# ai4ce/V2X-Sim

Measured on AMD Instinct MI355X. Metric: BEV frames/sec, V2VNet 5-agent detection (256x256 BEV), higher is better.
Workload: dtype bf16

## Files before the change

### v2x-sim_amd/csrc/api.hip

```cpp
#include "common.h"
#include <cxxabi.h>
#include <dlfcn.h>
#include <stdlib.h>
#include <string.h>

static thread_local char g_err[512] = "";

void v2x_set_error(const char *fmt, ...) {
    va_list ap;
    va_start(ap, fmt);
    vsnprintf(g_err, sizeof(g_err), fmt, ap);
    va_end(ap);
}

extern "C" __attribute__((weak)) int v2x_probe_build_marker;
extern "C" int v2x_abi_version(void) { return &v2x_probe_build_marker != nullptr ? -V2X_AMD_ABI_VERSION : V2X_AMD_ABI_VERSION; }

struct v2x_launch_plan { char *buf; size_t cap, len; };
__thread v2x_launch_plan *v2x_plan_sink = nullptr;

int v2x_plan_record(const void *kernel, const char *what) {
    v2x_launch_plan &p = *v2x_plan_sink;
    Dl_info info;
    char *dem = nullptr;
// ... 11 lines not shown
            else if (b[i] == '(' && --depth == 0) { n = i; break; }
        }
    }
    const size_t sep = p.len ? 3 : 0;
    const bool fits = p.len + sep + n + 1 <= p.cap;
    if (fits) {
        memcpy(p.buf + p.len, " + ", sep);
        memcpy(p.buf + p.len + sep, b, n);
        p.len += sep + n;
        p.buf[p.len] = 0;
    }
    free(dem);
    V2X_REQUIRE(fits, "v2x_conv2d_plan: the kernel names do not fit %zu bytes", p.cap);
    return V2X_OK;
}

extern "C" int v2x_conv2d_plan(const v2x_conv_desc *d, char *buf, size_t cap) {
    V2X_REQUIRE(buf && cap > 0, "v2x_conv2d_plan: no buffer");
    buf[0] = 0;
    v2x_launch_plan plan = {buf, cap, 0};
    v2x_plan_sink = &plan;
    const int rc = v2x_conv2d(d, nullptr);
    v2x_plan_sink = nullptr;
    return rc;
}

#include <atomic>
#include <mutex>
#include <strings.h>
namespace {
struct TuneEntry { const char *name; int def; };
const TuneEntry kTune[V2X_TUNE_COUNT] = {
    {"STREAM_WAVES", 8}, {"STREAM_G", 1}, {"STREAM_WT", 1}, {"STORE_X4", 1}, {"STREAM_PERSIST", 1}, {"STREAM_WIDE", 1},
    {"WIDE3", 1}, {"HALO_PP", 1}, {"VOXELIZE_LDS", 1}, {"WARP_LDS", 2}, {"S2_G", 1}, {"GRU_XCD_WALK", 1}, {"HALO_XCD", 1}, {"WGRAD_TR", 1}, {"BN_PARTIAL_T", 1}, {"WGRAD_REDUCE4", 1}, {"CONV1X1", 1},
};
std::atomic<int> g_tune[V2X_TUNE_COUNT];
std::once_flag g_tune_once;
void tune_init() {
    for (int i = 0; i < V2X_TUNE_COUNT; ++i) {
        char env[64];
        snprintf(env, sizeof(env), "V2X_%s", kTune[i].name);
        const char *e = getenv(env);
        g_tune[i].store((e && *e) ? atoi(e) : kTune[i].def, std::memory_order_relaxed);
    }
}
int tune_find(const char *name) {
    if (!name) return -1;
    if (strncasecmp(name, "V2X_", 4) == 0) name += 4;
    for (int i = 0; i < V2X_TUNE_COUNT; ++i)
        if (strcasecmp(name, kTune[i].name) == 0) return i;
    return -1;
}
}

int v2x_tune(int id) {
    std::call_once(g_tune_once, tune_init);
    return g_tune[id].load(std::memory_order_relaxed);
}
extern "C" int v2x_tuning_set(const char *name, int value) {
    const int i = tune_find(name);
    V2X_REQUIRE(i >= 0, "v2x_tuning_set: unknown switch '%s'", name ? name : "(null)");
    std::call_once(g_tune_once, tune_init);
    g_tune[i].store(value, std::memory_order_relaxed);
    return V2X_OK;
}
extern "C" int v2x_tuning_get(const char *name, int *value) {
    const int i = tune_find(name);
// ... 6 lines not shown
```

### v2x-sim_amd/csrc/common.h

```cpp
#pragma once
#include <hip/hip_runtime.h>
#include <stdint.h>
#include <stdio.h>
#include <stdarg.h>

#include "../../include/v2x_amd.h"

typedef __attribute__((ext_vector_type(8))) __bf16 bf16x8_t;
typedef __attribute__((ext_vector_type(4))) float f32x4_t;
typedef __attribute__((ext_vector_type(16))) float f32x16_t;

void v2x_set_error(const char *fmt, ...);

enum v2x_tune_id {
    V2X_TUNE_STREAM_WAVES,
    V2X_TUNE_STREAM_G,
    V2X_TUNE_STREAM_WT,
    V2X_TUNE_STORE_X4,
    V2X_TUNE_STREAM_PERSIST,
    V2X_TUNE_STREAM_WIDE,
    V2X_TUNE_WIDE3,
    V2X_TUNE_HALO_PP,
    V2X_TUNE_VOXELIZE_LDS,
    V2X_TUNE_WARP_LDS,
    V2X_TUNE_S2_G,
    V2X_TUNE_GRU_XCD_WALK,
    V2X_TUNE_HALO_XCD,
    V2X_TUNE_WGRAD_TR,
    V2X_TUNE_BN_PARTIAL_T,
    V2X_TUNE_WGRAD_REDUCE4,
    V2X_TUNE_CONV1X1,
    V2X_TUNE_COUNT
};
int v2x_tune(int id);

#define V2X_REQUIRE(cond, ...)            \
    do {                                  \
        if (!(cond)) {                    \
            v2x_set_error(__VA_ARGS__);   \
            return V2X_EINVAL;            \
        }                                 \
    } while (0)

#define V2X_CHECK_LAUNCH(name)                                                   \
    do {                                                                         \
        hipError_t e_ = hipGetLastError();                                       \
        if (e_ != hipSuccess) {                                                  \
            v2x_set_error("%s: launch failed: %s", name, hipGetErrorString(e_)); \
            return V2X_EIO;                                                      \
        }                                                                        \
    } while (0)

#define V2X_MAX_DEVICES 32
struct v2x_once_per_device { bool done[V2X_MAX_DEVICES]; };
static inline bool v2x_first_use_on_device(v2x_once_per_device &o) {
    int dev = 0;
    if (hipGetDevice(&dev) != hipSuccess || dev < 0 || dev >= V2X_MAX_DEVICES) return true;
    if (o.done[dev]) return false;
    o.done[dev] = true;
    return true;
}

struct v2x_launch_plan;
extern __thread v2x_launch_plan *v2x_plan_sink;
// ... 72 lines not shown
```

### v2x-sim_amd/csrc/conv_stream_pc.hip

```cpp
#include "conv_stream.h"

namespace pcs {
constexpr int TH = 16, TW = 32, BCO = 128, TCO = 8, HCO = 4;
constexpr int PW0 = TW / 2 + 2, PH0 = TH / 2 + 2;
constexpr int PHF = TH + 2, PWH = (TW + 2) / 2;
constexpr int SLICE = BCO * 64;
constexpr int USTEP = 4 * SLICE, SSTEP = 3 * SLICE;
constexpr int UP_PIECES = (PH0 * PW0 * 4 + 63) / 64;
constexpr int SP_PIECES = (2 * PHF * PWH * 4 + 63) / 64;
#ifndef V2X_PCS_USLOTS_BUILD
#define V2X_PCS_USLOTS_BUILD 3
#endif
constexpr int NU = V2X_PCS_USLOTS_BUILD;
constexpr int OFF_P0 = 3 * SSTEP, OFF_P1 = OFF_P0 + SP_PIECES * 1024;
constexpr int OFF_UPA = NU * USTEP, OFF_UPB = OFF_UPA + UP_PIECES * 1024;
constexpr int OFF_SS = (OFF_UPB + UP_PIECES * 1024 > OFF_P1 + SP_PIECES * 1024) ? OFF_UPB + UP_PIECES * 1024 : OFF_P1 + SP_PIECES * 1024;
constexpr int SMEM = OFF_SS + 2 * BCO * 4;
static_assert(SMEM <= 160 * 1024 && (NU == 3 || NU == 4), "LDS map");
#define PCS_SWZ(pc) (((pc) >> 1) & 3)

}

__global__ __launch_bounds__(512) __attribute__((amdgpu_waves_per_eu(2, 2))) void conv3x3_stream8p_kernel(const StreamArgs a) {
    using namespace pcs;
    extern __shared__ __attribute__((aligned(16))) char smem[];
    const int tid = threadIdx.x;
    const int lane = tid & 63;
    const int wave = __builtin_amdgcn_readfirstlane(tid >> 6);
    const int grp = wave >> 2, wv = wave & 3;
    const int py = wv >> 1, px = wv & 1;
    const int fj = lane & 15, fq = lane >> 4;

    const int nwg = gridDim.x;
    int bid = blockIdx.x;
    {
        const int q = nwg >> 3, r = nwg & 7, xcd = bid & 7, i = bid >> 3;
        bid = (xcd < r ? xcd * (q + 1) : r * (q + 1) + (xcd - r) * q) + i;
    }
    const int n_tiles = a.n_px_tiles * a.n_co_tiles;
    const int co_tile = bid % a.n_co_tiles;
    const int txy = a.tiles_x * a.tiles_y;
    const int n_up = a.C0 >> 5, n_sk = a.C1 >> 5;
    const int S_up = 4 * n_up, S_sk = 3 * n_sk;
    const size_t tile_bytes = (size_t)S_up * USTEP + (size_t)S_sk * SSTEP;
    const char *w_up = reinterpret_cast<const char *>(a.w) + (size_t)co_tile * tile_bytes;
    const char *w_sk = w_up + (size_t)S_up * USTEP;
    const void *zero_page = reinterpret_cast<const char *>(a.w) + (size_t)a.n_co_tiles * tile_bytes;
    const int Hs = a.H >> 1, Ws = a.W >> 1;

    auto tile_coords = [&](int t, int &n, int &y0, int &x0) {
        const int px_tile = t / a.n_co_tiles;
        n = px_tile / txy;
        const int trem = px_tile - n * txy;
        const int ty = trem / a.tiles_x;
        y0 = ty * TH;
        x0 = (trem - ty * a.tiles_x) * TW;
    };
    auto fresh_lane = [&]() -> int {
        int l;
        asm volatile("v_mbcnt_lo_u32_b32 %0, -1, 0\n\tv_mbcnt_hi_u32_b32 %0, -1, %0" : "=v"(l));
        return l;
    };
    auto issue_up_patch_piece = [&](int n, int y0, int x0, int kc, int piece, int buf_off) {
        const int L = piece * 64 + fresh_lane();
// ... 7 lines not shown
    auto issue_sk_patch_piece = [&](int n, int y0, int x0, int kc, int piece, int buf_off) {
        const int L = piece * 64 + fresh_lane();
        const int pix = L >> 2, phys = L & 3;
        const int q = pix / (PHF * PWH), rem = pix - q * (PHF * PWH);
        const int pr = rem / PWH, cc = rem - pr * PWH;
        const int y = y0 - 1 + pr, x = x0 - 1 + 2 * cc + q;
        const bool ok = pix < 2 * PHF * PWH && (unsigned)y < (unsigned)a.H && (unsigned)x < (unsigned)a.W;
        const unsigned off = (unsigned)((n * a.H + y) * a.W + x) * (unsigned)a.C1 + (unsigned)(kc * 32 + ((phys ^ PCS_SWZ(cc)) << 3));
        glds16s(ok ? (const void *)(a.in1 + off) : zero_page, smem + buf_off + piece * 1024);
    };
    auto issue_up_weights = [&](int st, int first, int count) {
        const int lane_w = fresh_lane();
        const char *src = w_up + (size_t)st * USTEP + lane_w * 16;
        char *dst = smem + (st % NU) * USTEP;
#pragma unroll
        for (int u = 0; u < 12; ++u)
            if (u < count) glds16s(src + (first + u) * 1024, dst + (first + u) * 1024);
    };
    auto issue_sk_weights = [&](int st, int first, int count) {
        const int lane_w = fresh_lane();
        const char *src = w_sk + (size_t)st * SSTEP + lane_w * 16;
        char *dst = smem + (st % 3) * SSTEP;
#pragma unroll
        for (int u = 0; u < 6; ++u)
            if (u < count) glds16s(src + (first + u) * 1024, dst + (first + u) * 1024);
    };
    auto up_buf = [&](int kc) { return ((n_up - 1 - kc) & 1) ? OFF_UPB : OFF_UPA; };
    auto sk_buf = [&](int kc) { return (kc & 1) ? OFF_P0 : OFF_P1; };
    auto up_prologue = [&](int n, int y0, int x0) {
        if (grp == 0) {
#pragma unroll
            for (int u = 0; u < 3; ++u) issue_up_patch_piece(n, y0, x0, 0, wv + 4 * u, up_buf(0));
        }
        if constexpr (NU == 3) {
            issue_up_weights(wave >> 2, (wave & 3) * 8, 8);
        } else {
            issue_up_weights((wave * 12) / 32, (wave * 12) % 32, ((wave * 12) % 32 + 12 <= 32) ? 12 : 32 - (wave * 12) % 32);
            if ((wave * 12) % 32 + 12 > 32) issue_up_weights((wave * 12) / 32 + 1, 0, (wave * 12) % 32 + 12 - 32);
        }
    };

    float *s_ss = reinterpret_cast<float *>(smem + OFF_SS);
    for (int i = tid; i < BCO; i += 512) {
        const int co = co_tile * BCO + i;
        s_ss[i] = co < a.Cout ? a.scale[co] : 0.f;
        s_ss[BCO + i] = co < a.Cout ? a.shift[co] : 0.f;
    }
    const uint32_t floor_bits = a.relu ? 0u : 0x80008000u;

    int tile = bid;
    int n, y0, x0;
    tile_coords(tile, n, y0, x0);
    up_prologue(n, y0, x0);
    asm volatile("s_waitcnt vmcnt(0) lgkmcnt(0)" ::: "memory");

    for (;;) {
        const int next = tile + nwg;
        const bool has_next = next < n_tiles;
        f32x4_t acc[TCO][4];
#pragma unroll
        for (int i = 0; i < TCO; ++i)
#pragma unroll
            for (int f = 0; f < 4; ++f) acc[i][f] = (f32x4_t)(0.f);

        __builtin_amdgcn_s_barrier();
        if (grp == 1) __builtin_amdgcn_s_barrier();
        for (int kc = 0; kc < n_up; ++kc) {
            const char *pb = smem + up_buf(kc);
#pragma unroll
            for (int t = 0; t < 4; ++t) {
                const int st = kc * 4 + t;
                const int ta = t >> 1, tb = t & 1;
                const int ln = fresh_lane();
                const int fjl = ln & 15, fql = ln >> 4;
                [[maybe_unused]] int nw = 0;
                if (grp == 1) {
                    if (st + NU - 1 < S_up) {
                        issue_up_weights(st + NU - 1, wv * 8, 8);
                        nw = 8;
                    }
                } else if (t < 3 && kc + 1 < n_up) {
                    issue_up_patch_piece(n, y0, x0, kc + 1, wv + 4 * t, up_buf(kc + 1));
                }
                __builtin_amdgcn_sched_barrier(0);
                bf16x8_t B[4], A[TCO];
                {
                    const int pc = fjl + tb + px;
                    const char *p = pb + ((4 * grp + py + ta) * PW0 * 4 + pc * 4 + (fql ^ PCS_SWZ(pc))) * 16;
#pragma unroll
                    for (int y = 0; y < 4; ++y) B[y] = *reinterpret_cast<const bf16x8_t *>(p + y * (PW0 * 64));
                    const char *ws = smem + (st % NU) * USTEP + wv * SLICE + (fql * BCO + fjl) * 16;
#pragma unroll
                    for (int i = 0; i < TCO; ++i) A[i] = *reinterpret_cast<const bf16x8_t *>(ws + i * 256);
                }
                __builtin_amdgcn_s_waitcnt(0xc07f);
                if (grp == 1) {
                    int keep = 0;
                    for (int d = 2; d <= NU - 1; ++d) keep += (st + d < S_up) ? 8 : 0;
                    const int stores = (st < NU - 2) ? (a.x4 ? 16 : 32) : 0;
                    switch (keep + stores) {
                        case 8: asm volatile("s_waitcnt vmcnt(8)" ::: "memory"); break;
                        case 16: asm volatile("s_waitcnt vmcnt(16)" ::: "memory"); break;
                        case 24: asm volatile("s_waitcnt vmcnt(24)" ::: "memory"); break;
                        case 32: asm volatile("s_waitcnt vmcnt(32)" ::: "memory"); break;
                        case 40: asm volatile("s_waitcnt vmcnt(40)" ::: "memory"); break;
                        case 48: asm volatile("s_waitcnt vmcnt(48)" ::: "memory"); break;
                        default: asm volatile("s_waitcnt vmcnt(0)" ::: "memory"); break;
                    }
                } else if (t == 3) {
                    asm volatile("s_waitcnt vmcnt(0)" ::: "memory");
                }
                __builtin_amdgcn_sched_barrier(0);
                __builtin_amdgcn_s_barrier();
                __builtin_amdgcn_sched_barrier(0);
#pragma unroll
                for (int i = 0; i < TCO; ++i)
#pragma unroll
                    for (int y = 0; y < 4; ++y) acc[i][y] = __builtin_amdgcn_mfma_f32_16x16x32_bf16(A[i], B[y], acc[i][y], 0, 0, 0);
                __builtin_amdgcn_sched_barrier(0);
                __builtin_amdgcn_s_barrier();
                __builtin_amdgcn_sched_barrier(0);
            }
        }
        if (grp == 0) __builtin_amdgcn_s_barrier();

        if (grp == 0) {
#pragma unroll
            for (int u = 0; u < 10; ++u)
                if (wv + 4 * u < SP_PIECES) issue_sk_patch_piece(n, y0, x0, 0, wv + 4 * u, sk_buf(0));
        }
        issue_sk_weights(wave >> 2, (wave & 3) * 6, 6);
        asm volatile("s_waitcnt vmcnt(0)" ::: "memory");
        __builtin_amdgcn_s_barrier();
        if (grp == 1) __builtin_amdgcn_s_barrier();
        for (int kc = 0; kc < n_sk; ++kc) {
            const char *pb = smem + sk_buf(kc);
#pragma unroll 1
            for (int kx = 0; kx < 3; ++kx) {
                const int st = kc * 3 + kx;
                const int ln = fresh_lane();
                const int fjl = ln & 15, fql = ln >> 4;
                int nw = 0;
                if (grp == 1) {
                    if (st + 2 < S_sk) {
                        issue_sk_weights(st + 2, wv * 6, 6);
                        nw = 6;
                    }
                } else if (kx < 2 && kc + 1 < n_sk) {
#pragma unroll
                    for (int u = 0; u < 5; ++u) {
                        const int piece = wv + 4 * (kx * 5 + u);
                        if (piece < SP_PIECES) issue_sk_patch_piece(n, y0, x0, kc + 1, piece, sk_buf(kc + 1));
                    }
                }
// ... 22 lines not shown
                for (int h = 0; h < 6; ++h) {
                    const int ky = h >> 1, hh = h & 1;
                    __builtin_amdgcn_sched_barrier(0);
#pragma unroll
                    for (int y = 0; y < 4; ++y) acc[hh * HCO][y] = __builtin_amdgcn_mfma_f32_16x16x32_bf16(A[h & 1][0], B[2 * y + ky], acc[hh * HCO][y], 0, 0, 0);
                    __builtin_amdgcn_sched_barrier(0);
                    if (h + 1 < 6) {
                        const int ky1 = (h + 1) >> 1, hh1 = (h + 1) & 1;
#pragma unroll
                        for (int i = 0; i < HCO; ++i) A[(h + 1) & 1][i] = *reinterpret_cast<const bf16x8_t *>(ws + ky1 * SLICE + (hh1 * HCO + i) * 256);
                    }
                    __builtin_amdgcn_sched_barrier(0);
#pragma unroll
                    for (int i = 1; i < HCO; ++i)
#pragma unroll
                        for (int y = 0; y < 4; ++y)
                            acc[hh * HCO + i][y] = __builtin_amdgcn_mfma_f32_16x16x32_bf16(A[h & 1][i], B[2 * y + ky], acc[hh * HCO + i][y], 0, 0, 0);
                    __builtin_amdgcn_sched_barrier(0);
                }
                __builtin_amdgcn_sched_barrier(0);
                __builtin_amdgcn_s_barrier();
                __builtin_amdgcn_sched_barrier(0);
            }
        }
        if (grp == 0) __builtin_amdgcn_s_barrier();

        int nn = 0, ny0 = 0, nx0 = 0;
        if (has_next) {
            tile_coords(next, nn, ny0, nx0);
            up_prologue(nn, ny0, nx0);
        }
        {
            lds_cf_t *lss = (lds_cf_t *)s_ss;
#pragma unroll
            for (int i = 0; i < TCO; i += 2) {
                float4 sc[2], sf[2];
#pragma unroll
                for (int h = 0; h < 2; ++h) {
                    sc[h] = lds_ld4(lss + (i + h) * 16 + fq * 4);
                    sf[h] = lds_ld4(lss + BCO + (i + h) * 16 + fq * 4);
                }
#pragma unroll
                for (int y = 0; y < 4; ++y) {
                    uint32_t ox[2], oy[2];
#pragma unroll
                    for (int h = 0; h < 2; ++h) {
                        ox[h] = v2x_relu_bf16x2_floor(pack_bf16x2(acc[i + h][y][0] * sc[h].x + sf[h].x, acc[i + h][y][1] * sc[h].y + sf[h].y), floor_bits);
                        oy[h] = v2x_relu_bf16x2_floor(pack_bf16x2(acc[i + h][y][2] * sc[h].z + sf[h].z, acc[i + h][y][3] * sc[h].w + sf[h].w), floor_bits);
                    }
                    const size_t pix = (size_t)(n * a.H + y0 + 8 * grp + 2 * y + py) * a.W + x0 + 2 * fj + px;
                    uint16_t *p = reinterpret_cast<uint16_t *>(a.out) + pix * a.out_cstride + a.out_coff + co_tile * BCO + i * 16 + fq * 4;
                    if (a.x4) {
                        v2x_store_pair_x4(p, fq, ox[0], oy[0], ox[1], oy[1]);
                    } else {
                        *reinterpret_cast<uint2 *>(p) = make_uint2(ox[0], oy[0]);
                        *reinterpret_cast<uint2 *>(p + 16) = make_uint2(ox[1], oy[1]);
                    }
                }
            }
        }
        if (!has_next) break;
        if (a.x4) asm volatile("s_waitcnt vmcnt(16)" ::: "memory");
        else asm volatile("s_waitcnt vmcnt(32)" ::: "memory");
        tile = next;
        n = nn;
        y0 = ny0;
        x0 = nx0;
    }
}

namespace pcq {
constexpr int BCO = 64, TCO = 4;
constexpr int SLICE = BCO * 64;
constexpr int USTEP = 4 * SLICE, SSTEP = 3 * SLICE;
constexpr int OFF_UP = 3 * USTEP;
constexpr int OFF_SP = 3 * SSTEP;
constexpr int OFF_SS = OFF_SP + 2 * pcs::SP_PIECES * 1024, SMEM = OFF_SS + 2 * BCO * 4;
static_assert(OFF_UP + 4 * pcs::UP_PIECES * 1024 <= OFF_SS && SMEM <= 160 * 1024, "LDS map");
}

__global__ __launch_bounds__(512) __attribute__((amdgpu_waves_per_eu(2, 2))) void conv3x3_stream8q_kernel(const StreamArgs a) {
    using namespace pcq;
    using pcs::PW0; using pcs::PH0; using pcs::PHF; using pcs::PWH; using pcs::UP_PIECES; using pcs::SP_PIECES; using pcs::TH;
    extern __shared__ __attribute__((aligned(16))) char smem[];
    const int tid = threadIdx.x;
    const int lane = tid & 63;
    const int wave = __builtin_amdgcn_readfirstlane(tid >> 6);
    const int grp = wave >> 2, wv = wave & 3;
    const int py = wv >> 1, px = wv & 1;
    const int fj = lane & 15, fq = lane >> 4;
    const int nwg = gridDim.x;
    int bid = blockIdx.x;
    {
        const int q = nwg >> 3, r = nwg & 7, xcd = bid & 7, i = bid >> 3;
        bid = (xcd < r ? xcd * (q + 1) : r * (q + 1) + (xcd - r) * q) + i;
    }
    const int n_tiles = a.n_px_tiles;
    const int txy = a.tiles_x * a.tiles_y;
    const int n_up = a.C0 >> 5, n_sk = a.C1 >> 5;
    const int S_up = 4 * n_up, S_sk = 3 * n_sk;
    const char *w_up = reinterpret_cast<const char *>(a.w);
    const char *w_sk = w_up + (size_t)S_up * USTEP;
    const void *zero_page = w_sk + (size_t)S_sk * SSTEP;
    const int Hs = a.H >> 1, Ws = a.W >> 1;

    auto tile_coords = [&](int t, int &n, int &y0, int &x0) {
        n = t / txy;
        const int trem = t - n * txy;
        const int ty = trem / a.tiles_x;
        y0 = ty * TH;
        x0 = (trem - ty * a.tiles_x) * 64 + 32 * grp;
    };
    auto fresh_lane = [&]() -> int {
        int l;
        asm volatile("v_mbcnt_lo_u32_b32 %0, -1, 0\n\tv_mbcnt_hi_u32_b32 %0, -1, %0" : "=v"(l));
        return l;
    };
    auto issue_up_patch_piece = [&](int n, int y0, int x0, int kc, int piece, int buf_off) {
        const int L = piece * 64 + fresh_lane();
        const int pix = L >> 2, phys = L & 3;
        const int pr = pix / PW0, pc = pix - pr * PW0;
        const int y = (y0 >> 1) - 1 + pr, x = (x0 >> 1) - 1 + pc;
        const bool ok = pix < PH0 * PW0 && (unsigned)y < (unsigned)Hs && (unsigned)x < (unsigned)Ws;
        const unsigned off = (unsigned)((n * Hs + y) * Ws + x) * (unsigned)a.C0 + (unsigned)(kc * 32 + ((phys ^ PCS_SWZ(pc)) << 3));
        glds16s(ok ? (const void *)(a.in0 + off) : zero_page, smem + buf_off + piece * 1024);
    };
    auto issue_sk_patch_piece = [&](int n, int y0, int x0, int kc, int piece, int buf_off) {
        const int L = piece * 64 + fresh_lane();
        const int pix = L >> 2, phys = L & 3;
        const int q = pix / (PHF * PWH), rem = pix - q * (PHF * PWH);
        const int pr = rem / PWH, cc = rem - pr * PWH;
        const int y = y0 - 1 + pr, x = x0 - 1 + 2 * cc + q;
        const bool ok = pix < 2 * PHF * PWH && (unsigned)y < (unsigned)a.H && (unsigned)x < (unsigned)a.W;
        const unsigned off = (unsigned)((n * a.H + y) * a.W + x) * (unsigned)a.C1 + (unsigned)(kc * 32 + ((phys ^ PCS_SWZ(cc)) << 3));
        glds16s(ok ? (const void *)(a.in1 + off) : zero_page, smem + buf_off + piece * 1024);
    };
    auto issue_up_weights = [&](int st, int first, int count) {
        const int lane_w = fresh_lane();
        const char *src = w_up + (size_t)st * USTEP + lane_w * 16;
        char *dst = smem + (st % 3) * USTEP;
#pragma unroll
        for (int u = 0; u < 4; ++u)
            if (u < count) glds16s(src + (first + u) * 1024, dst + (first + u) * 1024);
    };
    auto issue_sk_weights = [&](int st, int first, int count) {
        const int lane_w = fresh_lane();
        const char *src = w_sk + (size_t)st * SSTEP + lane_w * 16;
        char *dst = smem + (st % 3) * SSTEP;
#pragma unroll
        for (int u = 0; u < 3; ++u)
            if (u < count) glds16s(src + (first + u) * 1024, dst + (first + u) * 1024);
    };
    auto up_buf = [&](int kc) { return OFF_UP + (grp * 2 + (kc & 1)) * (UP_PIECES * 1024); };
    const int sk_buf = OFF_SP + grp * (SP_PIECES * 1024);
    auto up_prologue = [&](int n, int y0, int x0) {
#pragma unroll
        for (int u = 0; u < 3; ++u) issue_up_patch_piece(n, y0, x0, 0, wv + 4 * u, up_buf(0));
        issue_up_weights(wave >> 2, (wave & 3) * 4, 4);
    };

    float *s_ss = reinterpret_cast<float *>(smem + OFF_SS);
    for (int i = tid; i < BCO; i += 512) {
        s_ss[i] = i < a.Cout ? a.scale[i] : 0.f;
        s_ss[BCO + i] = i < a.Cout ? a.shift[i] : 0.f;
    }
    const uint32_t floor_bits = a.relu ? 0u : 0x80008000u;

    int tile = bid;
    int n, y0, x0;
    tile_coords(tile, n, y0, x0);
    up_prologue(n, y0, x0);
    asm volatile("s_waitcnt vmcnt(0) lgkmcnt(0)" ::: "memory");

    for (;;) {
        const int next = tile + nwg;
        const bool has_next = next < n_tiles;
        f32x4_t acc[TCO][8];
#pragma unroll
        for (int i = 0; i < TCO; ++i)
#pragma unroll
            for (int f = 0; f < 8; ++f) acc[i][f] = (f32x4_t)(0.f);

        __builtin_amdgcn_s_barrier();
        if (grp == 1) __builtin_amdgcn_s_barrier();
        for (int kc = 0; kc < n_up; ++kc) {
            const char *pb = smem + up_buf(kc);
#pragma unroll
            for (int t = 0; t < 4; ++t) {
                const int st = kc * 4 + t;
                const int ta = t >> 1, tb = t & 1;
                const int ln = fresh_lane();
                const int fjl = ln & 15, fql = ln >> 4;
                int keep = 0;
                if (grp == 1 && st + 2 < S_up) {
                    issue_up_weights(st + 2, wv * 4, 4);
                    keep = 4;
                }
                if (t < 3 && kc + 1 < n_up) {
                    issue_up_patch_piece(n, y0, x0, kc + 1, wv + 4 * t, up_buf(kc + 1));
                    keep += 1;
                }
                __builtin_amdgcn_sched_barrier(0);
                bf16x8_t B[8], A[TCO];
                {
                    const int pc = fjl + tb + px;
                    const char *p = pb + ((py + ta) * PW0 * 4 + pc * 4 + (fql ^ PCS_SWZ(pc))) * 16;
#pragma unroll
                    for (int y = 0; y < 8; ++y) B[y] = *reinterpret_cast<const bf16x8_t *>(p + y * (PW0 * 64));
                    const char *ws = smem + (st % 3) * USTEP + wv * SLICE + (fql * BCO + fjl) * 16;
#pragma unroll
                    for (int i = 0; i < TCO; ++i) A[i] = *reinterpret_cast<const bf16x8_t *>(ws + i * 256);
                }
                __builtin_amdgcn_s_waitcnt(0xc07f);
                if (grp == 1) {
                    const int nst = st == 0 ? (a.x4 ? 16 : 32) : 0;
                    switch (keep + nst) {
                        case 1: asm volatile("s_waitcnt vmcnt(1)" ::: "memory"); break;
                        case 4: asm volatile("s_waitcnt vmcnt(4)" ::: "memory"); break;
                        case 5: asm volatile("s_waitcnt vmcnt(5)" ::: "memory"); break;
                        case 21: asm volatile("s_waitcnt vmcnt(21)" ::: "memory"); break;
                        case 37: asm volatile("s_waitcnt vmcnt(37)" ::: "memory"); break;
                        default: asm volatile("s_waitcnt vmcnt(0)" ::: "memory"); break;
                    }
                } else if (t == 3) {
                    asm volatile("s_waitcnt vmcnt(0)" ::: "memory");
                }
                __builtin_amdgcn_sched_barrier(0);
                __builtin_amdgcn_s_barrier();
                __builtin_amdgcn_sched_barrier(0);
#pragma unroll
                for (int i = 0; i < TCO; ++i)
#pragma unroll
                    for (int y = 0; y < 8; ++y) acc[i][y] = __builtin_amdgcn_mfma_f32_16x16x32_bf16(A[i], B[y], acc[i][y], 0, 0, 0);
                __builtin_amdgcn_sched_barrier(0);
                __builtin_amdgcn_s_barrier();
                __builtin_amdgcn_sched_barrier(0);
            }
        }
        if (grp == 0) __builtin_amdgcn_s_barrier();

#pragma unroll
        for (int u = 0; u < 10; ++u)
            if (wv + 4 * u < SP_PIECES) issue_sk_patch_piece(n, y0, x0, 0, wv + 4 * u, sk_buf);
        issue_sk_weights(wave >> 2, (wave & 3) * 3, 3);
        asm volatile("s_waitcnt vmcnt(0)" ::: "memory");
        __builtin_amdgcn_s_barrier();
        if (grp == 1) __builtin_amdgcn_s_barrier();
        for (int kc = 0; kc < n_sk; ++kc) {
            const char *pb = smem + sk_buf;
            if (kc > 0) {
#pragma unroll
                for (int u = 0; u < 10; ++u)
                    if (wv + 4 * u < SP_PIECES) issue_sk_patch_piece(n, y0, x0, kc, wv + 4 * u, sk_buf);
                asm volatile("s_waitcnt vmcnt(0)" ::: "memory");
                __builtin_amdgcn_s_barrier();
            }
#pragma unroll 1
            for (int kx = 0; kx < 3; ++kx) {
                const int st = kc * 3 + kx;
                const int ln = fresh_lane();
                const int fjl = ln & 15, fql = ln >> 4;
                int nw = 0;
                if (grp == 1 && st + 2 < S_sk) {
                    issue_sk_weights(st + 2, wv * 3, 3);
                    nw = 3;
                }
                __builtin_amdgcn_sched_barrier(0);
                bf16x8_t B[9], A[3][TCO];
                const char *ws = smem + (st % 3) * SSTEP + (fql * BCO + fjl) * 16;
// ... 14 lines not shown
                __builtin_amdgcn_s_barrier();
                __builtin_amdgcn_sched_barrier(0);
#pragma unroll
                for (int ky = 0; ky < 3; ++ky)
#pragma unroll
                    for (int i = 0; i < TCO; ++i)
#pragma unroll
                        for (int y = 0; y < 4; ++y) acc[i][y] = __builtin_amdgcn_mfma_f32_16x16x32_bf16(A[ky][i], B[2 * y + ky], acc[i][y], 0, 0, 0);
                __builtin_amdgcn_sched_barrier(0);
#pragma unroll
                for (int r = 0; r < 9; ++r) B[r] = *reinterpret_cast<const bf16x8_t *>(p + (8 + r) * (PWH * 64));
                __builtin_amdgcn_s_waitcnt(0xc07f);
                __builtin_amdgcn_sched_barrier(0);
#pragma unroll
                for (int ky = 0; ky < 3; ++ky)
#pragma unroll
                    for (int i = 0; i < TCO; ++i)
#pragma unroll
                        for (int y = 0; y < 4; ++y) acc[i][4 + y] = __builtin_amdgcn_mfma_f32_16x16x32_bf16(A[ky][i], B[2 * y + ky], acc[i][4 + y], 0, 0, 0);
                __builtin_amdgcn_sched_barrier(0);
                __builtin_amdgcn_s_barrier();
                __builtin_amdgcn_sched_barrier(0);
            }
        }
        if (grp == 0) __builtin_amdgcn_s_barrier();

        int nn = 0, ny0 = 0, nx0 = 0;
        if (has_next) {
            tile_coords(next, nn, ny0, nx0);
            up_prologue(nn, ny0, nx0);
        }
        {
            lds_cf_t *lss = (lds_cf_t *)s_ss;
#pragma unroll
            for (int i = 0; i < TCO; i += 2) {
                float4 sc[2], sf[2];
#pragma unroll
                for (int h = 0; h < 2; ++h) {
                    sc[h] = lds_ld4(lss + (i + h) * 16 + fq * 4);
                    sf[h] = lds_ld4(lss + BCO + (i + h) * 16 + fq * 4);
                }
#pragma unroll
                for (int y = 0; y < 8; ++y) {
                    uint32_t ox[2], oy[2];
#pragma unroll
                    for (int h = 0; h < 2; ++h) {
                        ox[h] = v2x_relu_bf16x2_floor(pack_bf16x2(acc[i + h][y][0] * sc[h].x + sf[h].x, acc[i + h][y][1] * sc[h].y + sf[h].y), floor_bits);
                        oy[h] = v2x_relu_bf16x2_floor(pack_bf16x2(acc[i + h][y][2] * sc[h].z + sf[h].z, acc[i + h][y][3] * sc[h].w + sf[h].w), floor_bits);
                    }
                    const size_t pix = (size_t)(n * a.H + y0 + 2 * y + py) * a.W + x0 + 2 * fj + px;
                    uint16_t *p = reinterpret_cast<uint16_t *>(a.out) + pix * a.out_cstride + a.out_coff + i * 16 + fq * 4;
                    if (a.x4) {
                        v2x_store_pair_x4(p, fq, ox[0], oy[0], ox[1], oy[1]);
                    } else {
                        *reinterpret_cast<uint2 *>(p) = make_uint2(ox[0], oy[0]);
                        *reinterpret_cast<uint2 *>(p + 16) = make_uint2(ox[1], oy[1]);
                    }
                }
            }
        }
        if (!has_next) break;
        if (a.x4) asm volatile("s_waitcnt vmcnt(16)" ::: "memory");
        else asm volatile("s_waitcnt vmcnt(32)" ::: "memory");
        tile = next;
        n = nn;
        y0 = ny0;
        x0 = nx0;
    }
}

int v2x_conv_stream_pc_launch(const StreamArgs &a, hipStream_t s) {
    if (a.Cout == 64) {
        int grid = a.n_px_tiles;
        const int g = v2x_num_cus();
        if (g > 0 && g < grid) grid = g;
        return v2x_launch<conv3x3_stream8q_kernel>("conv3x3_stream8q_kernel", dim3(grid), dim3(512), pcq::SMEM, s, a);
    }
    const int n_tiles = a.n_px_tiles * a.n_co_tiles;
    int grid = n_tiles;
    const int g = v2x_num_cus() / a.n_co_tiles * a.n_co_tiles;
    if (g > 0 && g < n_tiles) grid = g;
    return v2x_launch<conv3x3_stream8p_kernel>("conv3x3_stream8p_kernel", dim3(grid), dim3(512), pcs::SMEM, s, a);
}
```

### v2x-sim_amd/v2x_sim_amd/tuning.py

```python
import ctypes as C
import os

_HOST_DEFAULTS = {"CONV_PAIR": 1, "TRAIN_HIP": 1, "TRAIN_GRAPH": 1, "TRAIN_HIP_CONV": 0, "SMALL_BATCH": 2, "WARP_HIP": 1, "WARP_XCD": 1, "SEG_FUSE": 1, "TRAIN_PACK_BATCH": 1, "TRAIN_LOSS_HIP": 1, "TRAIN_GATES_HIP": 1, "PARITY_CLASS": 3, "TAIL_FUSE": 1, "TRAIN_HEAD_PACK": 1, "TRAIN_BN_BIAS_ZERO": 1, "TRAIN_UPCAT_CONV": 1, "TRAIN_SPLITK": 480, "TRAIN_V2V_NHWC": 1, "TRAIN_ADAM_HIP": 1, "SPLITK_TARGET": 320,
                  "TRAIN_SEG_LOSS_HIP": 0, "TRAIN_SEG_HEAD_FUSE": 0, "TRAIN_SEG_GRAPH": 0}
LIBRARY_SWITCHES = ("STREAM_WAVES", "STREAM_G", "STREAM_WT", "STORE_X4", "STREAM_PERSIST", "STREAM_WIDE", "WIDE3", "HALO_PP",
                    "VOXELIZE_LDS", "WARP_LDS", "S2_G", "GRU_XCD_WALK", "HALO_XCD", "WGRAD_TR", "BN_PARTIAL_T", "WGRAD_REDUCE4", "CONV1X1")


def _env_int(name, default):
    v = os.environ.get("V2X_" + name, "")
    try:
        return int(v) if v != "" else default
    except ValueError:
        return default


_host = {k: _env_int(k, d) for k, d in _HOST_DEFAULTS.items()}


def _norm(name):
    name = name.upper()
    return name[4:] if name.startswith("V2X_") else name


def get(name):
    name = _norm(name)
    if name in _host:
        return _host[name]
    from . import _lib
    out = C.c_int(0)
    _lib.check(_lib.load().v2x_tuning_get(name.encode(), C.byref(out)), "v2x_tuning_get(%s)" % name)
    return out.value


def set(name, value):
    name = _norm(name)
    old = get(name)
    if name in _host:
        _host[name] = int(value)
# ... 5 lines not shown
```

Measured before the change: 6599.

## Process two up-path taps per barrier in stream conv kernels

Templates the stream8p/stream8q conv kernels on taps per step. The new default path handles two horizontal taps per synchronisation round, using four weight slots and interleaving the second tap's LDS loads with the first tap's MFMAs. This halves the number of workgroup barriers and vmcnt waits in the up-path loop. In exchange it uses more registers (extra A/B fragments) and more LDS, and the old single-tap kernels stay selectable through a new UP_TAPS2 switch.

```diff
diff --git a/v2x-sim_amd/csrc/api.hip b/v2x-sim_amd/csrc/api.hip
--- a/v2x-sim_amd/csrc/api.hip
+++ b/v2x-sim_amd/csrc/api.hip
@@ -67,7 +67,7 @@
 struct TuneEntry { const char *name; int def; };
 const TuneEntry kTune[V2X_TUNE_COUNT] = {
     {"STREAM_WAVES", 8}, {"STREAM_G", 1}, {"STREAM_WT", 1}, {"STORE_X4", 1}, {"STREAM_PERSIST", 1}, {"STREAM_WIDE", 1},
-    {"WIDE3", 1}, {"HALO_PP", 1}, {"VOXELIZE_LDS", 1}, {"WARP_LDS", 2}, {"S2_G", 1}, {"GRU_XCD_WALK", 1}, {"HALO_XCD", 1}, {"WGRAD_TR", 1}, {"BN_PARTIAL_T", 1}, {"WGRAD_REDUCE4", 1}, {"CONV1X1", 1},
+    {"WIDE3", 1}, {"HALO_PP", 1}, {"VOXELIZE_LDS", 1}, {"WARP_LDS", 2}, {"S2_G", 1}, {"GRU_XCD_WALK", 1}, {"HALO_XCD", 1}, {"WGRAD_TR", 1}, {"BN_PARTIAL_T", 1}, {"WGRAD_REDUCE4", 1}, {"CONV1X1", 1}, {"UP_TAPS2", 2},
 };
 std::atomic<int> g_tune[V2X_TUNE_COUNT];
 std::once_flag g_tune_once;
diff --git a/v2x-sim_amd/csrc/common.h b/v2x-sim_amd/csrc/common.h
--- a/v2x-sim_amd/csrc/common.h
+++ b/v2x-sim_amd/csrc/common.h
@@ -30,6 +30,7 @@
     V2X_TUNE_BN_PARTIAL_T,
     V2X_TUNE_WGRAD_REDUCE4,
     V2X_TUNE_CONV1X1,
+    V2X_TUNE_UP_TAPS2,
     V2X_TUNE_COUNT
 };
 int v2x_tune(int id);
diff --git a/v2x-sim_amd/csrc/conv_stream_pc.hip b/v2x-sim_amd/csrc/conv_stream_pc.hip
--- a/v2x-sim_amd/csrc/conv_stream_pc.hip
+++ b/v2x-sim_amd/csrc/conv_stream_pc.hip
@@ -8,28 +8,28 @@
 constexpr int USTEP = 4 * SLICE, SSTEP = 3 * SLICE;
 constexpr int UP_PIECES = (PH0 * PW0 * 4 + 63) / 64;
 constexpr int SP_PIECES = (2 * PHF * PWH * 4 + 63) / 64;
-#ifndef V2X_PCS_USLOTS_BUILD
-#define V2X_PCS_USLOTS_BUILD 3
-#endif
-constexpr int NU = V2X_PCS_USLOTS_BUILD;
-constexpr int OFF_P0 = 3 * SSTEP, OFF_P1 = OFF_P0 + SP_PIECES * 1024;
-constexpr int OFF_UPA = NU * USTEP, OFF_UPB = OFF_UPA + UP_PIECES * 1024;
-constexpr int OFF_SS = (OFF_UPB + UP_PIECES * 1024 > OFF_P1 + SP_PIECES * 1024) ? OFF_UPB + UP_PIECES * 1024 : OFF_P1 + SP_PIECES * 1024;
-constexpr int SMEM = OFF_SS + 2 * BCO * 4;
-static_assert(SMEM <= 160 * 1024 && (NU == 3 || NU == 4), "LDS map");
+template <int UT>
+struct Map {
+    static constexpr int NU = UT == 2 ? 4 : 3;
+    static constexpr int OFF_P0 = 3 * SSTEP, OFF_P1 = OFF_P0 + SP_PIECES * 1024;
+    static constexpr int OFF_UPA = NU * USTEP, OFF_UPB = OFF_UPA + UP_PIECES * 1024;
+    static constexpr int OFF_SS = (OFF_UPB + UP_PIECES * 1024 > OFF_P1 + SP_PIECES * 1024) ? OFF_UPB + UP_PIECES * 1024 : OFF_P1 + SP_PIECES * 1024;
+    static constexpr int SMEM = OFF_SS + 2 * BCO * 4;
+    static_assert(SMEM <= 160 * 1024, "LDS map");
+};
 #define PCS_SWZ(pc) (((pc) >> 1) & 3)
 
 }
 
-__global__ __launch_bounds__(512) __attribute__((amdgpu_waves_per_eu(2, 2))) void conv3x3_stream8p_kernel(const StreamArgs a) {
+template <int UT>
+__device__ __forceinline__ void stream8p_body(const StreamArgs &a) {
     using namespace pcs;
+    constexpr int NU = Map<UT>::NU, OFF_P0 = Map<UT>::OFF_P0, OFF_P1 = Map<UT>::OFF_P1, OFF_UPA = Map<UT>::OFF_UPA, OFF_UPB = Map<UT>::OFF_UPB, OFF_SS = Map<UT>::OFF_SS;
     extern __shared__ __attribute__((aligned(16))) char smem[];
     const int tid = threadIdx.x;
-    const int lane = tid & 63;
     const int wave = __builtin_amdgcn_readfirstlane(tid >> 6);
     const int grp = wave >> 2, wv = wave & 3;
     const int py = wv >> 1, px = wv & 1;
-    const int fj = lane & 15, fq = lane >> 4;
 
     const int nwg = gridDim.x;
     int bid = blockIdx.x;
@@ -103,12 +103,7 @@
 #pragma unroll
             for (int u = 0; u < 3; ++u) issue_up_patch_piece(n, y0, x0, 0, wv + 4 * u, up_buf(0));
         }
-        if constexpr (NU == 3) {
-            issue_up_weights(wave >> 2, (wave & 3) * 8, 8);
-        } else {
-            issue_up_weights((wave * 12) / 32, (wave * 12) % 32, ((wave * 12) % 32 + 12 <= 32) ? 12 : 32 - (wave * 12) % 32);
-            if ((wave * 12) % 32 + 12 > 32) issue_up_weights((wave * 12) / 32 + 1, 0, (wave * 12) % 32 + 12 - 32);
-        }
+        issue_up_weights(wave >> 2, (wave & 3) * 8, 8);
     };
 
     float *s_ss = reinterpret_cast<float *>(smem + OFF_SS);
@@ -136,61 +131,121 @@
 
         __builtin_amdgcn_s_barrier();
         if (grp == 1) __builtin_amdgcn_s_barrier();
-        for (int kc = 0; kc < n_up; ++kc) {
-            const char *pb = smem + up_buf(kc);
-#pragma unroll
-            for (int t = 0; t < 4; ++t) {
-                const int st = kc * 4 + t;
-                const int ta = t >> 1, tb = t & 1;
-                const int ln = fresh_lane();
-                const int fjl = ln & 15, fql = ln >> 4;
-                [[maybe_unused]] int nw = 0;
-                if (grp == 1) {
-                    if (st + NU - 1 < S_up) {
-                        issue_up_weights(st + NU - 1, wv * 8, 8);
-                        nw = 8;
-                    }
-                } else if (t < 3 && kc + 1 < n_up) {
-                    issue_up_patch_piece(n, y0, x0, kc + 1, wv + 4 * t, up_buf(kc + 1));
-                }
-                __builtin_amdgcn_sched_barrier(0);
-                bf16x8_t B[4], A[TCO];
-                {
-                    const int pc = fjl + tb + px;
-                    const char *p = pb + ((4 * grp + py + ta) * PW0 * 4 + pc * 4 + (fql ^ PCS_SWZ(pc))) * 16;
-#pragma unroll
-                    for (int y = 0; y < 4; ++y) B[y] = *reinterpret_cast<const bf16x8_t *>(p + y * (PW0 * 64));
-                    const char *ws = smem + (st % NU) * USTEP + wv * SLICE + (fql * BCO + fjl) * 16;
-#pragma unroll
-                    for (int i = 0; i < TCO; ++i) A[i] = *reinterpret_cast<const bf16x8_t *>(ws + i * 256);
-                }
-                __builtin_amdgcn_s_waitcnt(0xc07f);
-                if (grp == 1) {
-                    int keep = 0;
-                    for (int d = 2; d <= NU - 1; ++d) keep += (st + d < S_up) ? 8 : 0;
-                    const int stores = (st < NU - 2) ? (a.x4 ? 16 : 32) : 0;
-                    switch (keep + stores) {
-                        case 8: asm volatile("s_waitcnt vmcnt(8)" ::: "memory"); break;
-                        case 16: asm volatile("s_waitcnt vmcnt(16)" ::: "memory"); break;
-                        case 24: asm volatile("s_waitcnt vmcnt(24)" ::: "memory"); break;
-                        case 32: asm volatile("s_waitcnt vmcnt(32)" ::: "memory"); break;
-                        case 40: asm volatile("s_waitcnt vmcnt(40)" ::: "memory"); break;
-                        case 48: asm volatile("s_waitcnt vmcnt(48)" ::: "memory"); break;
-                        default: asm volatile("s_waitcnt vmcnt(0)" ::: "memory"); break;
-                    }
-                } else if (t == 3) {
+        if constexpr (UT == 2) {
+            for (int kc = 0; kc < n_up; ++kc) {
+                const char *pb = smem + up_buf(kc);
+#pragma unroll 1
+                for (int ta = 0; ta < 2; ++ta) {
+                    const int tp = kc * 4 + 2 * ta;
+                    if (tp + 2 < S_up) issue_up_weights(tp + 2 + grp, wv * 8, 8);
+                    if (grp == 0 && ta == 1 && kc + 1 < n_up) {
+#pragma unroll
+                        for (int u = 0; u < 3; ++u) issue_up_patch_piece(n, y0, x0, kc + 1, wv + 4 * u, up_buf(kc + 1));
+                    }
+                    __builtin_amdgcn_sched_barrier(0);
+                    bf16x8_t B0[4], B1[4], A[TCO], A1[TCO];
+                    {
+                        const int ln = fresh_lane();
+                        const int fjl = ln & 15, fql = ln >> 4;
+                        const int pc = fjl + px;
+                        const char *p = pb + ((4 * grp + py + ta) * PW0 * 4 + pc * 4 + (fql ^ PCS_SWZ(pc))) * 16;
+#pragma unroll
+                        for (int y = 0; y < 4; ++y) B0[y] = *reinterpret_cast<const bf16x8_t *>(p + y * (PW0 * 64));
+                        const char *ws = smem + (2 * ta) * USTEP + wv * SLICE + (fql * BCO + fjl) * 16;
+#pragma unroll
+                        for (int i = 0; i < TCO; ++i) A[i] = *reinterpret_cast<const bf16x8_t *>(ws + i * 256);
+                        const char *p1 = pb + ((4 * grp + py + ta) * PW0 * 4 + (pc + 1) * 4 + (fql ^ PCS_SWZ(pc + 1))) * 16;
+#pragma unroll
+                        for (int y = 0; y < 4; ++y) B1[y] = *reinterpret_cast<const bf16x8_t *>(p1 + y * (PW0 * 64));
+                    }
+                    __builtin_amdgcn_s_waitcnt(0xc07f);
+                    __builtin_amdgcn_sched_barrier(0);
+                    __builtin_amdgcn_s_barrier();
+                    __builtin_amdgcn_sched_barrier(0);
+                    {
+                        const int ln = fresh_lane();
+                        const int fjl = ln & 15, fql = ln >> 4;
+                        const char *ws1 = smem + (2 * ta + 1) * USTEP + wv * SLICE + (fql * BCO + fjl) * 16;
+                        A1[TCO - 2] = *reinterpret_cast<const bf16x8_t *>(ws1 + (TCO - 2) * 256);
+                        A1[TCO - 1] = *reinterpret_cast<const bf16x8_t *>(ws1 + (TCO - 1) * 256);
+                        __builtin_amdgcn_sched_barrier(0);
+#pragma unroll
+                        for (int i = 0; i < TCO; ++i) {
+#pragma unroll
+                            for (int y = 0; y < 4; ++y) acc[i][y] = __builtin_amdgcn_mfma_f32_16x16x32_bf16(A[i], B0[y], acc[i][y], 0, 0, 0);
+                            __builtin_amdgcn_sched_barrier(0);
+                            if (i < TCO - 2) A1[i] = *reinterpret_cast<const bf16x8_t *>(ws1 + i * 256);
+                            __builtin_amdgcn_sched_barrier(0);
+                        }
+#pragma unroll
+                        for (int i = 0; i < TCO; ++i)
+#pragma unroll
+                            for (int y = 0; y < 4; ++y) acc[i][y] = __builtin_amdgcn_mfma_f32_16x16x32_bf16(A1[i], B1[y], acc[i][y], 0, 0, 0);
+                        __builtin_amdgcn_sched_barrier(0);
+                    }
                     asm volatile("s_waitcnt vmcnt(0)" ::: "memory");
-                }
-                __builtin_amdgcn_sched_barrier(0);
-                __builtin_amdgcn_s_barrier();
-                __builtin_amdgcn_sched_barrier(0);
-#pragma unroll
-                for (int i = 0; i < TCO; ++i)
-#pragma unroll
-                    for (int y = 0; y < 4; ++y) acc[i][y] = __builtin_amdgcn_mfma_f32_16x16x32_bf16(A[i], B[y], acc[i][y], 0, 0, 0);
-                __builtin_amdgcn_sched_barrier(0);
-                __builtin_amdgcn_s_barrier();
-                __builtin_amdgcn_sched_barrier(0);
+                    __builtin_amdgcn_sched_barrier(0);
+                    __builtin_amdgcn_s_barrier();
+                    __builtin_amdgcn_sched_barrier(0);
+                }
+            }
+        } else {
+            for (int kc = 0; kc < n_up; ++kc) {
+                const char *pb = smem + up_buf(kc);
+#pragma unroll
+                for (int t = 0; t < 4; ++t) {
+                    const int st = kc * 4 + t;
+                    const int ta = t >> 1, tb = t & 1;
+                    const int ln = fresh_lane();
+                    const int fjl = ln & 15, fql = ln >> 4;
+                    [[maybe_unused]] int nw = 0;
+                    if (grp == 1) {
+                        if (st + NU - 1 < S_up) {
+                            issue_up_weights(st + NU - 1, wv * 8, 8);
+                            nw = 8;
+                        }
+                    } else if (t < 3 && kc + 1 < n_up) {
+                        issue_up_patch_piece(n, y0, x0, kc + 1, wv + 4 * t, up_buf(kc + 1));
+                    }
+                    __builtin_amdgcn_sched_barrier(0);
+                    bf16x8_t B[4], A[TCO];
+                    {
+                        const int pc = fjl + tb + px;
+                        const char *p = pb + ((4 * grp + py + ta) * PW0 * 4 + pc * 4 + (fql ^ PCS_SWZ(pc))) * 16;
+#pragma unroll
+                        for (int y = 0; y < 4; ++y) B[y] = *reinterpret_cast<const bf16x8_t *>(p + y * (PW0 * 64));
+                        const char *ws = smem + (st % NU) * USTEP + wv * SLICE + (fql * BCO + fjl) * 16;
+#pragma unroll
+                        for (int i = 0; i < TCO; ++i) A[i] = *reinterpret_cast<const bf16x8_t *>(ws + i * 256);
+                    }
+                    __builtin_amdgcn_s_waitcnt(0xc07f);
+                    if (grp == 1) {
+                        int keep = 0;
+                        for (int d = 2; d <= NU - 1; ++d) keep += (st + d < S_up) ? 8 : 0;
+                        const int stores = (st < NU - 2) ? (a.x4 ? 16 : 32) : 0;
+                        switch (keep + stores) {
+                            case 8: asm volatile("s_waitcnt vmcnt(8)" ::: "memory"); break;
+                            case 16: asm volatile("s_waitcnt vmcnt(16)" ::: "memory"); break;
+                            case 24: asm volatile("s_waitcnt vmcnt(24)" ::: "memory"); break;
+                            case 32: asm volatile("s_waitcnt vmcnt(32)" ::: "memory"); break;
+                            case 40: asm volatile("s_waitcnt vmcnt(40)" ::: "memory"); break;
+                            case 48: asm volatile("s_waitcnt vmcnt(48)" ::: "memory"); break;
+                            default: asm volatile("s_waitcnt vmcnt(0)" ::: "memory"); break;
+                        }
+                    } else if (t == 3) {
+                        asm volatile("s_waitcnt vmcnt(0)" ::: "memory");
+                    }
+                    __builtin_amdgcn_sched_barrier(0);
+                    __builtin_amdgcn_s_barrier();
+                    __builtin_amdgcn_sched_barrier(0);
+#pragma unroll
+                    for (int i = 0; i < TCO; ++i)
+#pragma unroll
+                        for (int y = 0; y < 4; ++y) acc[i][y] = __builtin_amdgcn_mfma_f32_16x16x32_bf16(A[i], B[y], acc[i][y], 0, 0, 0);
+                    __builtin_amdgcn_sched_barrier(0);
+                    __builtin_amdgcn_s_barrier();
+                    __builtin_amdgcn_sched_barrier(0);
+                }
             }
         }
         if (grp == 0) __builtin_amdgcn_s_barrier();
@@ -279,6 +334,8 @@
         }
         {
             lds_cf_t *lss = (lds_cf_t *)s_ss;
+            const int le = fresh_lane();
+            const int fj = le & 15, fq = le >> 4;
 #pragma unroll
             for (int i = 0; i < TCO; i += 2) {
                 float4 sc[2], sf[2];
@@ -316,26 +373,33 @@
     }
 }
 
+__global__ __launch_bounds__(512) __attribute__((amdgpu_waves_per_eu(2, 2))) void conv3x3_stream8p_kernel(const StreamArgs a) { stream8p_body<2>(a); }
+__global__ __launch_bounds__(512) __attribute__((amdgpu_waves_per_eu(2, 2))) void conv3x3_stream8p_1tap_kernel(const StreamArgs a) { stream8p_body<1>(a); }
+
 namespace pcq {
 constexpr int BCO = 64, TCO = 4;
 constexpr int SLICE = BCO * 64;
 constexpr int USTEP = 4 * SLICE, SSTEP = 3 * SLICE;
-constexpr int OFF_UP = 3 * USTEP;
 constexpr int OFF_SP = 3 * SSTEP;
 constexpr int OFF_SS = OFF_SP + 2 * pcs::SP_PIECES * 1024, SMEM = OFF_SS + 2 * BCO * 4;
-static_assert(OFF_UP + 4 * pcs::UP_PIECES * 1024 <= OFF_SS && SMEM <= 160 * 1024, "LDS map");
+template <int UT>
+struct Map {
+    static constexpr int NU = UT == 2 ? 4 : 3;
+    static constexpr int OFF_UP = NU * USTEP;
+    static_assert(OFF_UP + 4 * pcs::UP_PIECES * 1024 <= OFF_SS && SMEM <= 160 * 1024, "LDS map");
+};
 }
 
-__global__ __launch_bounds__(512) __attribute__((amdgpu_waves_per_eu(2, 2))) void conv3x3_stream8q_kernel(const StreamArgs a) {
+template <int UT>
+__device__ __forceinline__ void stream8q_body(const StreamArgs &a) {
     using namespace pcq;
+    constexpr int NU = Map<UT>::NU, OFF_UP = Map<UT>::OFF_UP;
     using pcs::PW0; using pcs::PH0; using pcs::PHF; using pcs::PWH; using pcs::UP_PIECES; using pcs::SP_PIECES; using pcs::TH;
     extern __shared__ __attribute__((aligned(16))) char smem[];
     const int tid = threadIdx.x;
-    const int lane = tid & 63;
     const int wave = __builtin_amdgcn_readfirstlane(tid >> 6);
     const int grp = wave >> 2, wv = wave & 3;
     const int py = wv >> 1, px = wv & 1;
-    const int fj = lane & 15, fq = lane >> 4;
     const int nwg = gridDim.x;
     int bid = blockIdx.x;
     {
@@ -385,7 +449,7 @@
     auto issue_up_weights = [&](int st, int first, int count) {
         const int lane_w = fresh_lane();
         const char *src = w_up + (size_t)st * USTEP + lane_w * 16;
-        char *dst = smem + (st % 3) * USTEP;
+        char *dst = smem + (st % NU) * USTEP;
 #pragma unroll
         for (int u = 0; u < 4; ++u)
             if (u < count) glds16s(src + (first + u) * 1024, dst + (first + u) * 1024);
@@ -430,58 +494,123 @@
 
         __builtin_amdgcn_s_barrier();
         if (grp == 1) __builtin_amdgcn_s_barrier();
-        for (int kc = 0; kc < n_up; ++kc) {
-            const char *pb = smem + up_buf(kc);
-#pragma unroll
-            for (int t = 0; t < 4; ++t) {
-                const int st = kc * 4 + t;
-                const int ta = t >> 1, tb = t & 1;
-                const int ln = fresh_lane();
-                const int fjl = ln & 15, fql = ln >> 4;
-                int keep = 0;
-                if (grp == 1 && st + 2 < S_up) {
-                    issue_up_weights(st + 2, wv * 4, 4);
-                    keep = 4;
-                }
-                if (t < 3 && kc + 1 < n_up) {
-                    issue_up_patch_piece(n, y0, x0, kc + 1, wv + 4 * t, up_buf(kc + 1));
-                    keep += 1;
-                }
-                __builtin_amdgcn_sched_barrier(0);
-                bf16x8_t B[8], A[TCO];
-                {
-                    const int pc = fjl + tb + px;
-                    const char *p = pb + ((py + ta) * PW0 * 4 + pc * 4 + (fql ^ PCS_SWZ(pc))) * 16;
-#pragma unroll
-                    for (int y = 0; y < 8; ++y) B[y] = *reinterpret_cast<const bf16x8_t *>(p + y * (PW0 * 64));
-                    const char *ws = smem + (st % 3) * USTEP + wv * SLICE + (fql * BCO + fjl) * 16;
-#pragma unroll
-                    for (int i = 0; i < TCO; ++i) A[i] = *reinterpret_cast<const bf16x8_t *>(ws + i * 256);
-                }
-                __builtin_amdgcn_s_waitcnt(0xc07f);
-                if (grp == 1) {
-                    const int nst = st == 0 ? (a.x4 ? 16 : 32) : 0;
-                    switch (keep + nst) {
-                        case 1: asm volatile("s_waitcnt vmcnt(1)" ::: "memory"); break;
-                        case 4: asm volatile("s_waitcnt vmcnt(4)" ::: "memory"); break;
-                        case 5: asm volatile("s_waitcnt vmcnt(5)" ::: "memory"); break;
-                        case 21: asm volatile("s_waitcnt vmcnt(21)" ::: "memory"); break;
-                        case 37: asm volatile("s_waitcnt vmcnt(37)" ::: "memory"); break;
-                        default: asm volatile("s_waitcnt vmcnt(0)" ::: "memory"); break;
-                    }
-                } else if (t == 3) {
+        if constexpr (UT == 2) {
+            for (int kc = 0; kc < n_up; ++kc) {
+                const char *pb = smem + up_buf(kc);
+#pragma unroll 1
+                for (int ta = 0; ta < 2; ++ta) {
+                    const int tp = kc * 4 + 2 * ta;
+                    if (tp + 2 < S_up) issue_up_weights(tp + 2 + grp, wv * 4, 4);
+                    if (kc + 1 < n_up) {
+                        if (ta == 0) {
+                            issue_up_patch_piece(n, y0, x0, kc + 1, wv, up_buf(kc + 1));
+                            issue_up_patch_piece(n, y0, x0, kc + 1, wv + 4, up_buf(kc + 1));
+                        } else {
+                            issue_up_patch_piece(n, y0, x0, kc + 1, wv + 8, up_buf(kc + 1));
+                        }
+                    }
+                    __builtin_amdgcn_sched_barrier(0);
+                    bf16x8_t B[8], B1[8], A[TCO], A1[TCO];
+                    {
+                        const int ln = fresh_lane();
+                        const int fjl = ln & 15, fql = ln >> 4;
+                        const int pc = fjl + px;
+                        const char *p = pb + ((py + ta) * PW0 * 4 + pc * 4 + (fql ^ PCS_SWZ(pc))) * 16;
+#pragma unroll
+                        for (int y = 0; y < 8; ++y) B[y] = *reinterpret_cast<const bf16x8_t *>(p + y * (PW0 * 64));
+                        const char *ws = smem + (2 * ta) * USTEP + wv * SLICE + (fql * BCO + fjl) * 16;
+#pragma unroll
+                        for (int i = 0; i < TCO; ++i) A[i] = *reinterpret_cast<const bf16x8_t *>(ws + i * 256);
+                    }
+                    __builtin_amdgcn_s_waitcnt(0xc07f);
+                    __builtin_amdgcn_sched_barrier(0);
+                    __builtin_amdgcn_s_barrier();
+                    __builtin_amdgcn_sched_barrier(0);
+                    {
+                        const int ln = fresh_lane();
+                        const int fjl = ln & 15, fql = ln >> 4;
+                        const int pc1 = fjl + px + 1;
+                        const char *p1 = pb + ((py + ta) * PW0 * 4 + pc1 * 4 + (fql ^ PCS_SWZ(pc1))) * 16;
+                        const char *ws1 = smem + (2 * ta + 1) * USTEP + wv * SLICE + (fql * BCO + fjl) * 16;
+#pragma unroll
+                        for (int i = 0; i < TCO; ++i) A1[i] = *reinterpret_cast<const bf16x8_t *>(ws1 + i * 256);
+                        B1[6] = *reinterpret_cast<const bf16x8_t *>(p1 + 6 * (PW0 * 64));
+                        B1[7] = *reinterpret_cast<const bf16x8_t *>(p1 + 7 * (PW0 * 64));
+                        __builtin_amdgcn_sched_barrier(0);
+#pragma unroll
+                        for (int y = 0; y < 8; ++y) {
+#pragma unroll
+                            for (int i = 0; i < TCO; ++i) acc[i][y] = __builtin_amdgcn_mfma_f32_16x16x32_bf16(A[i], B[y], acc[i][y], 0, 0, 0);
+                            __builtin_amdgcn_sched_barrier(0);
+                            if (y < 6) B1[y] = *reinterpret_cast<const bf16x8_t *>(p1 + y * (PW0 * 64));
+                            __builtin_amdgcn_sched_barrier(0);
+                        }
+#pragma unroll
+                        for (int i = 0; i < TCO; ++i)
+#pragma unroll
+                            for (int y = 0; y < 8; ++y) acc[i][y] = __builtin_amdgcn_mfma_f32_16x16x32_bf16(A1[i], B1[y], acc[i][y], 0, 0, 0);
+                        __builtin_amdgcn_sched_barrier(0);
+                    }
                     asm volatile("s_waitcnt vmcnt(0)" ::: "memory");
-                }
-                __builtin_amdgcn_sched_barrier(0);
-                __builtin_amdgcn_s_barrier();
-                __builtin_amdgcn_sched_barrier(0);
-#pragma unroll
-                for (int i = 0; i < TCO; ++i)
-#pragma unroll
-                    for (int y = 0; y < 8; ++y) acc[i][y] = __builtin_amdgcn_mfma_f32_16x16x32_bf16(A[i], B[y], acc[i][y], 0, 0, 0);
-                __builtin_amdgcn_sched_barrier(0);
-                __builtin_amdgcn_s_barrier();
-                __builtin_amdgcn_sched_barrier(0);
+                    __builtin_amdgcn_sched_barrier(0);
+                    __builtin_amdgcn_s_barrier();
+                    __builtin_amdgcn_sched_barrier(0);
+                }
+            }
+        } else {
+            for (int kc = 0; kc < n_up; ++kc) {
+                const char *pb = smem + up_buf(kc);
+#pragma unroll
+                for (int t = 0; t < 4; ++t) {
+                    const int st = kc * 4 + t;
+                    const int ta = t >> 1, tb = t & 1;
+                    const int ln = fresh_lane();
+                    const int fjl = ln & 15, fql = ln >> 4;
+                    int keep = 0;
+                    if (grp == 1 && st + 2 < S_up) {
+                        issue_up_weights(st + 2, wv * 4, 4);
+                        keep = 4;
+                    }
+                    if (t < 3 && kc + 1 < n_up) {
+                        issue_up_patch_piece(n, y0, x0, kc + 1, wv + 4 * t, up_buf(kc + 1));
+                        keep += 1;
+                    }
+                    __builtin_amdgcn_sched_barrier(0);
+                    bf16x8_t B[8], A[TCO];
+                    {
+                        const int pc = fjl + tb + px;
+                        const char *p = pb + ((py + ta) * PW0 * 4 + pc * 4 + (fql ^ PCS_SWZ(pc))) * 16;
+#pragma unroll
+                        for (int y = 0; y < 8; ++y) B[y] = *reinterpret_cast<const bf16x8_t *>(p + y * (PW0 * 64));
+                        const char *ws = smem + (st % NU) * USTEP + wv * SLICE + (fql * BCO + fjl) * 16;
+#pragma unroll
+                        for (int i = 0; i < TCO; ++i) A[i] = *reinterpret_cast<const bf16x8_t *>(ws + i * 256);
+                    }
+                    __builtin_amdgcn_s_waitcnt(0xc07f);
+                    if (grp == 1) {
+                        const int nst = st == 0 ? (a.x4 ? 16 : 32) : 0;
+                        switch (keep + nst) {
+                            case 1: asm volatile("s_waitcnt vmcnt(1)" ::: "memory"); break;
+                            case 4: asm volatile("s_waitcnt vmcnt(4)" ::: "memory"); break;
+                            case 5: asm volatile("s_waitcnt vmcnt(5)" ::: "memory"); break;
+                            case 21: asm volatile("s_waitcnt vmcnt(21)" ::: "memory"); break;
+                            case 37: asm volatile("s_waitcnt vmcnt(37)" ::: "memory"); break;
+                            default: asm volatile("s_waitcnt vmcnt(0)" ::: "memory"); break;
+                        }
+                    } else if (t == 3) {
+                        asm volatile("s_waitcnt vmcnt(0)" ::: "memory");
+                    }
+                    __builtin_amdgcn_sched_barrier(0);
+                    __builtin_amdgcn_s_barrier();
+                    __builtin_amdgcn_sched_barrier(0);
+#pragma unroll
+                    for (int i = 0; i < TCO; ++i)
+#pragma unroll
+                        for (int y = 0; y < 8; ++y) acc[i][y] = __builtin_amdgcn_mfma_f32_16x16x32_bf16(A[i], B[y], acc[i][y], 0, 0, 0);
+                    __builtin_amdgcn_sched_barrier(0);
+                    __builtin_amdgcn_s_barrier();
+                    __builtin_amdgcn_sched_barrier(0);
+                }
             }
         }
         if (grp == 0) __builtin_amdgcn_s_barrier();
@@ -562,6 +691,8 @@
         }
         {
             lds_cf_t *lss = (lds_cf_t *)s_ss;
+            const int le = fresh_lane();
+            const int fj = le & 15, fq = le >> 4;
 #pragma unroll
             for (int i = 0; i < TCO; i += 2) {
                 float4 sc[2], sf[2];
@@ -599,16 +730,23 @@
     }
 }
 
+__global__ __launch_bounds__(512) __attribute__((amdgpu_waves_per_eu(2, 2))) void conv3x3_stream8q_kernel(const StreamArgs a) { stream8q_body<2>(a); }
+__global__ __launch_bounds__(512) __attribute__((amdgpu_waves_per_eu(2, 2))) void conv3x3_stream8q_1tap_kernel(const StreamArgs a) { stream8q_body<1>(a); }
+
 int v2x_conv_stream_pc_launch(const StreamArgs &a, hipStream_t s) {
     if (a.Cout == 64) {
         int grid = a.n_px_tiles;
         const int g = v2x_num_cus();
         if (g > 0 && g < grid) grid = g;
+        if (v2x_tune(V2X_TUNE_UP_TAPS2) < 2)
+            return v2x_launch<conv3x3_stream8q_1tap_kernel>("conv3x3_stream8q_1tap_kernel", dim3(grid), dim3(512), pcq::SMEM, s, a);
         return v2x_launch<conv3x3_stream8q_kernel>("conv3x3_stream8q_kernel", dim3(grid), dim3(512), pcq::SMEM, s, a);
     }
     const int n_tiles = a.n_px_tiles * a.n_co_tiles;
     int grid = n_tiles;
     const int g = v2x_num_cus() / a.n_co_tiles * a.n_co_tiles;
     if (g > 0 && g < n_tiles) grid = g;
-    return v2x_launch<conv3x3_stream8p_kernel>("conv3x3_stream8p_kernel", dim3(grid), dim3(512), pcs::SMEM, s, a);
+    if (v2x_tune(V2X_TUNE_UP_TAPS2) == 0)
+        return v2x_launch<conv3x3_stream8p_1tap_kernel>("conv3x3_stream8p_1tap_kernel", dim3(grid), dim3(512), pcs::Map<1>::SMEM, s, a);
+    return v2x_launch<conv3x3_stream8p_kernel>("conv3x3_stream8p_kernel", dim3(grid), dim3(512), pcs::Map<2>::SMEM, s, a);
 }
diff --git a/v2x-sim_amd/v2x_sim_amd/tuning.py b/v2x-sim_amd/v2x_sim_amd/tuning.py
--- a/v2x-sim_amd/v2x_sim_amd/tuning.py
+++ b/v2x-sim_amd/v2x_sim_amd/tuning.py
@@ -4,7 +4,7 @@
 _HOST_DEFAULTS = {"CONV_PAIR": 1, "TRAIN_HIP": 1, "TRAIN_GRAPH": 1, "TRAIN_HIP_CONV": 0, "SMALL_BATCH": 2, "WARP_HIP": 1, "WARP_XCD": 1, "SEG_FUSE": 1, "TRAIN_PACK_BATCH": 1, "TRAIN_LOSS_HIP": 1, "TRAIN_GATES_HIP": 1, "PARITY_CLASS": 3, "TAIL_FUSE": 1, "TRAIN_HEAD_PACK": 1, "TRAIN_BN_BIAS_ZERO": 1, "TRAIN_UPCAT_CONV": 1, "TRAIN_SPLITK": 480, "TRAIN_V2V_NHWC": 1, "TRAIN_ADAM_HIP": 1, "SPLITK_TARGET": 320,
                   "TRAIN_SEG_LOSS_HIP": 0, "TRAIN_SEG_HEAD_FUSE": 0, "TRAIN_SEG_GRAPH": 0}
 LIBRARY_SWITCHES = ("STREAM_WAVES", "STREAM_G", "STREAM_WT", "STORE_X4", "STREAM_PERSIST", "STREAM_WIDE", "WIDE3", "HALO_PP",
-                    "VOXELIZE_LDS", "WARP_LDS", "S2_G", "GRU_XCD_WALK", "HALO_XCD", "WGRAD_TR", "BN_PARTIAL_T", "WGRAD_REDUCE4", "CONV1X1")
+                    "VOXELIZE_LDS", "WARP_LDS", "S2_G", "GRU_XCD_WALK", "HALO_XCD", "WGRAD_TR", "BN_PARTIAL_T", "WGRAD_REDUCE4", "CONV1X1", "UP_TAPS2")
 
 
 def _env_int(name, default):
```

Result: no change. 6651 (median of 6 runs) (+0.8%).
